# feldroop/genedex

Measured on AMD Instinct MI355X. Metric: queries/sec (count+locate), hg38-scale text, 100M len-50 reads, higher is better.
Workload: dtype u32

## Files before the change

### genedex_amd/csrc/search.hip

```cpp
#include <atomic>
#include <cstdlib>
#include <string>
#include <type_traits>

#include "common.hpp"
#include "kernels.hpp"

namespace gdx {

namespace {

constexpr int kBlock = 256;

struct QueryWindow {
    const uint64_t *words;
    uint64_t cur;
    uint64_t next;
    uint64_t cur_word;
    uint64_t first_word;

    __device__ __forceinline__ void init(const uint8_t *qbuf, uint64_t begin, uint64_t pos)
    {
        words = reinterpret_cast<const uint64_t *>(qbuf);
        first_word = begin >> 3;
// ... 1814 lines not shown
                    b[0] = a[0];
                    b[1] = a[1];
                }
                bool stepped = false;
                if (two) {
                    const uint32_t pair = (c2 - 1u) * 4u + (c1 - 1u);
                    const uint32_t bits_x = (c1 & 1u) | ((c1 & 2u) << 7) | ((c1 & 4u) << 14) | ((c2 & 1u) << 24);
                    const uint32_t bits_y = ((c2 >> 1) & 1u) | ((c2 & 4u) << 6);
                    const uint32_t nx = ~(bits_x * 0xffu);
                    const uint32_t ny = ~(bits_y * 0xffu) & 0xffffu;
                    uint32_t plo = 0, phi = 0;
#pragma unroll
                    for (int k = 0; k < 2; k++) {
                        plo += PairTable::pair_partial(a[k], sub + k * kGroup, pair, nx, ny, lo);
                        phi += PairTable::pair_partial(b[k], sub + k * kGroup, pair, nx, ny, hi);
                    }
                    const uint32_t nlo = quad_sum(plo), nhi = quad_sum(phi);
                    if (nlo != nhi) {
                        lo = nlo;
                        hi = nhi;
                        rem -= 2u;
                        part += 2u;
                        stepped = true;
                    }
                }
                if (!stepped) {
                    const uint32_t bits_x = (c1 & 1u) | ((c1 & 2u) << 7) | ((c1 & 4u) << 14);
                    const uint32_t nx = ~(bits_x * 0xffu) & 0xffffffu;
                    uint32_t plo = 0, phi = 0;
#pragma unroll
                    for (int k = 0; k < 2; k++) {
                        plo += PairTable::single_partial(a[k], sub + k * kGroup, c1, nx, lo);
                        phi += PairTable::single_partial(b[k], sub + k * kGroup, c1, nx, hi);
                    }
                    lo = quad_sum(plo);
                    hi = quad_sum(phi);
                    rem -= 1u;
                    part += 1u;
                }
                shift += part >> 3;
                part &= 7u;
            }
            if (writer) {
                if (bail) {
                    s_left[atomicAdd(&s_nleft, 1u)] = q;
                } else {
                    const bool unchanged = kCursor && len == 0u;
                    if (out_start && !unchanged) out_start[q] = lo;
                    if (out_end && !unchanged) out_end[q] = hi;
                    if (out_count) out_count[q] = hi - lo;
                    if (!kCursor && out_status) out_status[q] = 0;
                    if (kCursor && ca.active_out != nullptr && lo != hi && more_left) s_alive[slot] = q;
                }
            }
        }
        }
        __syncthreads();
        const uint32_t n_left = s_nleft;
        if (threadIdx.x == 0 && n_left != 0u) s_left_base = atomicAdd(n_leftover, n_left);
        __syncthreads();
        for (uint32_t i = threadIdx.x; i < n_left; i += kBlock) leftover[s_left_base + i] = s_left[i];
        __syncthreads();
        if (threadIdx.x == 0) s_nleft = 0;
        if (kCursor && ca.active_out != nullptr)
            flush_live_ordered(s_alive, cnt, s_alive_part, &s_alive_base, ca.active_out, ca.n_active_out);
    }
}

struct VerifyView {
    const uint2 *top;
    const u32x4 *text_units;
    const uint32_t *sa_full;
    const void *jump;
    const u32x4 *lines;
    const uint32_t *sb_offsets, *count, *sa_samples, *border_keys, *border_vals;
    const uint8_t *io_to_dense;
    uint32_t top_depth, n, n_texts, sa_inv, sa_rot, sa_limit, max_rows;
    uint32_t perm_code_lo, perm_code_hi, perm_exp_lo, perm_exp_hi, perm_mask;
    const u32x4 *seed;
    uint32_t seed_buckets, seed_k, seed_tag_bits;
    const u32x4 *seed_pairs, *seed_quads;
};

template <int kXlate, bool kSeed>
__global__ __launch_bounds__(kBlock) __attribute__((amdgpu_waves_per_eu(7, 7))) void search_verify_kernel4(
    VerifyView vv, const uint8_t *__restrict__ qbuf, const uint64_t *__restrict__ qbeg, const uint64_t *__restrict__ qend,
    uint64_t nq, uint32_t *__restrict__ out_count, uint8_t *__restrict__ out_status, uint4 *out_rec,
    uint32_t range, uint32_t *__restrict__ leftover, uint32_t *__restrict__ n_leftover,
    const uint32_t *__restrict__ list, const uint32_t *__restrict__ n_list,
    uint32_t ulen,
    const uint4 *state,
    uint32_t wide_to_list,
    uint32_t state_packed)
{
    constexpr int kGroup = 4;
    __shared__ uint8_t s_dense[256];
    __shared__ uint32_t s_count[8];
    __shared__ uint32_t s_left[kMaxRange];
    __shared__ uint32_t s_nleft, s_left_base;
    if (list != nullptr) nq = *n_list;
    if (static_cast<uint64_t>(blockIdx.x) * range >= nq) return;
    if (kXlate == 0)
        for (int i = threadIdx.x; i < 256; i += kBlock) s_dense[i] = vv.io_to_dense[i];
    if (threadIdx.x < 8) s_count[threadIdx.x] = threadIdx.x < 6 ? vv.count[threadIdx.x] : 0u;
    if (threadIdx.x == 0) s_nleft = 0;
    __syncthreads();
    IndexView ix{};
    ix.lines = vv.lines;
    ix.sb_offsets = vv.sb_offsets;
    ix.sa_inv = vv.sa_inv;
    ix.sa_rot = vv.sa_rot;
    ix.sa_limit = vv.sa_limit;
    const bool writer = (threadIdx.x % kGroup) == 0;
    const uint32_t sub = threadIdx.x & (kGroup - 1u);
    const uint32_t depth = vv.top_depth;
    const uint64_t n_ranges = (nq + range - 1) / range;
    for (uint64_t rg = blockIdx.x; rg < n_ranges; rg += gridDim.x) {
        const uint64_t base = rg * range;
        const uint32_t cnt = nq - base < range ? static_cast<uint32_t>(nq - base) : range;
        for (uint32_t slot = threadIdx.x / kGroup; slot < cnt; slot += kBlock / kGroup) {
            const uint32_t q = list != nullptr ? list[base + slot] : static_cast<uint32_t>(base + slot);
            uint4 st = make_uint4(0u, 0u, 0u, 0u);
            if (kSeed && state != nullptr) st = state[q];
            const bool from_state = kSeed && state != nullptr && state_packed != 0u && wide_to_list != 0u && (st.y & kStatePacked) != 0u &&
                                    (st.y & kStateSymbolsMask) <= 32u;
            const uint64_t begin = from_state ? 0ull : query_begin(qbeg, ulen, q);
            const uint64_t len = from_state ? 0ull : query_end(qend, ulen, q) - begin;
            bool bail = from_state ? false
                                   : (kSeed ? !(len >= vv.seed_k && len < (1ull << 21)) : !(len >= 16u && len >= depth && len < (1ull << 21)));
            uint32_t lo = 0, hi = 0, rem = 0;
            const uint64_t *wbase = query_words<kXlate>(qbuf, begin);
            const uint32_t off0 = static_cast<uint32_t>(begin & 7u);
            FastWindow w = {0u, 0u, 0u, 0u, 0u, 8u};
            uint32_t shift = 0, part = 0;
            bool single = false;
            bool single_ok = false;
            uint32_t pos = 0;
            bool resumed = false;
            const uint64_t state_codes = (static_cast<uint64_t>(st.z) << 32) | st.w;
            if (from_state && (st.y & kStatePair) != 0u && (st.y >> kStateRowsShift) > 2u) {
                const u32x4 *qr = vv.seed_quads + 4ull * st.x;
                const u32x4 q0 = qr[0], q1 = qr[1], q2 = qr[2], q3 = qr[3];
                const uint32_t n_v = st.y & kStateSymbolsMask, rows_q = st.y >> kStateRowsShift;
                const uint64_t vm64 = n_v == 32u ? ~0ull : ~0ull << (2u * (32u - n_v));
                const uint32_t p_me = sel4(sub, q0.x, q0.y, q0.z, q0.w);
                const uint64_t t_me = (static_cast<uint64_t>(sel4(sub, q1.y, q1.w, q2.y, q2.w)) << 32) | sel4(sub, q1.x, q1.z, q2.x, q2.z);
                uint32_t alive_q = (sub < rows_q && ((state_codes ^ t_me) & vm64) == 0ull && p_me >= n_v) ? 1u << sub : 0u;
                alive_q |= static_cast<uint32_t>(__builtin_amdgcn_mov_dpp(static_cast<int>(alive_q), 0xB1, 0xF, 0xF, true));
                alive_q |= static_cast<uint32_t>(__builtin_amdgcn_mov_dpp(static_cast<int>(alive_q), 0x4E, 0xF, 0xF, true));
                if (writer) {
                    const uint32_t n_alive = static_cast<uint32_t>(__popc(alive_q));
                    uint4 rec;
                    if (n_alive == 0u) {
                        rec = make_uint4(0u, 0u, 0xffffffffu, 0u);
                    } else if (n_alive <= 2u) {
                        const uint32_t f = static_cast<uint32_t>(__builtin_ctz(alive_q));
                        const uint32_t h1 = sel4(f, q0.x, q0.y, q0.z, q0.w) - n_v;
                        if (n_alive == 1u) {
                            rec = make_uint4(0u, 1u, h1, kRecResolved);
                        } else {
                            const uint32_t g = static_cast<uint32_t>(__builtin_ctz(alive_q & (alive_q - 1u)));
                            const uint32_t h2 = sel4(g, q0.x, q0.y, q0.z, q0.w) - n_v;
                            rec = make_uint4(h2, h2 + 2u, h1, kRecResolved);
                        }
                    } else {
                        rec = make_uint4(q3.x, q3.x + n_alive, alive_q, (n_v & 0x1fffffu) | kRecMasked);
                    }
                    if (out_rec) out_rec[q] = rec;
                    if (out_count) out_count[q] = rec.y - rec.x;
                    if (out_status) out_status[q] = 0;
                }
                continue;
            }
            if (from_state && (st.y & kStatePair) != 0u) {
                const u32x4 *pr = vv.seed_pairs + 2ull * st.x;
                const u32x4 r0 = pr[0], r1 = pr[1];
                const uint32_t n_v = st.y & kStateSymbolsMask;
                const uint64_t vm64 = n_v == 32u ? ~0ull : ~0ull << (2u * (32u - n_v));
                const uint64_t t1 = (static_cast<uint64_t>(r0.w) << 32) | r0.z, t2 = (static_cast<uint64_t>(r1.y) << 32) | r1.x;
                const bool ok1 = ((state_codes ^ t1) & vm64) == 0ull && r0.x >= n_v, ok2 = ((state_codes ^ t2) & vm64) == 0ull && r0.y >= n_v;
                if (writer) {
                    const uint32_t h1 = r0.x - n_v, h2 = r0.y - n_v;
                    uint4 rec;
                    if (ok1 && ok2) rec = make_uint4(h2, h2 + 2u, h1, kRecResolved);
                    else if (ok1 || ok2) rec = make_uint4(0u, 1u, ok1 ? h1 : h2, kRecResolved);
                    else rec = make_uint4(0u, 0u, 0xffffffffu, 0u);
                    if (out_rec) out_rec[q] = rec;
                    if (out_count) out_count[q] = rec.y - rec.x;
                    if (out_status) out_status[q] = 0;
                }
                continue;
            }
            if (from_state) {
                resumed = true;
                lo = st.x;
                hi = lo + (st.y >> kStateRowsShift);
                rem = st.y & kStateSymbolsMask;
            } else if (kSeed && !bail && state != nullptr) {
                const bool plain = state_packed == 0u && st.w == 1u;
                const bool p_rows = state_packed != 0u && (st.y & kStatePacked) != 0u, p_wide = state_packed != 0u && (st.y & kStatePlain) != 0u;
                if (plain || p_rows || p_wide) {
                    resumed = true;
                    rem = static_cast<uint32_t>(len);
                    w = fast_window<kXlate>(vv, s_dense, wbase, off0, rem, sub);
                    lo = st.x;
                    hi = plain ? st.y : (p_rows ? lo + (st.y >> kStateRowsShift) : st.z);
                    rem = plain ? st.z : st.y & kStateSymbolsMask;
                    shift = vv.seed_k >> 3;
                    part = vv.seed_k & 7u;
                }
            }
            if (kSeed && !bail && !resumed) {
                rem = static_cast<uint32_t>(len);
                w = fast_window<kXlate>(vv, s_dense, wbase, off0, rem, sub);
                const uint32_t k = vv.seed_k;
                const uint32_t n_look = rem < k + 32u ? rem : k + 32u;
                const uint32_t n_words = n_look <= w.s0 ? 1u : 1u + ((n_look - w.s0 + 7u) >> 3);
                if ((w.valid8 & ((1u << n_words) - 1u)) != (1u << n_words) - 1u) {
                    bail = true;
                } else {
                    const uint32_t w0 = __builtin_amdgcn_alignbit(w.l0, w.l0, 16), w1 = __builtin_amdgcn_alignbit(w.l1, w.l1, 16);
                    const uint32_t w2 = __builtin_amdgcn_alignbit(w.l2, w.l2, 16), w3 = __builtin_amdgcn_alignbit(w.l3, w.l3, 16);
                    const uint64_t key = ((static_cast<uint64_t>(w0) << 32) | w1) >> (64u - 2u * k);
                    uint32_t tag;
                    uint32_t b = seed_home(key, vv.seed_tag_bits, vv.seed_buckets, tag);
                    uint32_t ex, ey, ez, ew;
                    for (uint32_t d = 0;; d++) {
                        const u32x4 *bp = vv.seed + (static_cast<uint64_t>(b) << 3) + 2u * sub;
                        const u32x4 e0 = bp[0], e1 = bp[1];
                        const uint32_t want = tag | (d << kSeedDispShift);
                        const bool m0 = (e0.x & kSeedMatchMask) == want, m1 = (e1.x & kSeedMatchMask) == want;
                        const u32x4 es = m0 ? e0 : e1;
                        const bool m = m0 || m1;
                        ex = m ? (es.x | kSeedFound) : (e0.x & kSeedOverflow);
                        ey = m ? es.y : 0u;
                        ez = m ? es.z : 0u;
                        ew = m ? es.w : 0u;
                        ex |= static_cast<uint32_t>(__builtin_amdgcn_mov_dpp(static_cast<int>(ex), 0xB1, 0xF, 0xF, true));
                        ey |= static_cast<uint32_t>(__builtin_amdgcn_mov_dpp(static_cast<int>(ey), 0xB1, 0xF, 0xF, true));
                        ez |= static_cast<uint32_t>(__builtin_amdgcn_mov_dpp(static_cast<int>(ez), 0xB1, 0xF, 0xF, true));
                        ew |= static_cast<uint32_t>(__builtin_amdgcn_mov_dpp(static_cast<int>(ew), 0xB1, 0xF, 0xF, true));
                        ex |= static_cast<uint32_t>(__builtin_amdgcn_mov_dpp(static_cast<int>(ex), 0x4E, 0xF, 0xF, true));
                        ey |= static_cast<uint32_t>(__builtin_amdgcn_mov_dpp(static_cast<int>(ey), 0x4E, 0xF, 0xF, true));
                        ez |= static_cast<uint32_t>(__builtin_amdgcn_mov_dpp(static_cast<int>(ez), 0x4E, 0xF, 0xF, true));
                        ew |= static_cast<uint32_t>(__builtin_amdgcn_mov_dpp(static_cast<int>(ew), 0x4E, 0xF, 0xF, true));
                        if ((ex & kSeedFound) != 0u || (ex & kSeedOverflow) == 0u || d >= kSeedMaxDisp) break;
                        b = b + 1u == vv.seed_buckets ? 0u : b + 1u;
                    }
                    rem -= k;
                    shift = k >> 3;
                    part = k & 7u;
                    if ((ex & kSeedFound) == 0u) {
                        lo = hi = 0u;
                    } else if ((ex & kSeedKind) != 0u) {
                        lo = ey;
                        hi = ez;
                    } else {
                        single = true;
                        lo = 0u;
                        hi = 1u;
                        pos = ey;
                        uint32_t qh, ql;
                        const uint32_t sh = 32u - 2u * (k & 15u);
                        if (k == 16u) {
                            qh = w1;
                            ql = w2;
                        } else if (k < 16u) {
                            qh = __builtin_amdgcn_alignbit(w0, w1, sh);
                            ql = __builtin_amdgcn_alignbit(w1, w2, sh);
                        } else {
                            qh = __builtin_amdgcn_alignbit(w1, w2, sh);
                            ql = __builtin_amdgcn_alignbit(w2, w3, sh);
                        }
// ... 820 lines not shown
                    const uint32_t n_need = (static_cast<uint32_t>(at & 7u) + n_c + 7u) >> 3;
                    uint64_t lo64 = up[0];
                    uint32_t hi16 = 0;
                    if (n_need > 1u) lo64 |= static_cast<uint64_t>(up[1]) << 16;
                    if (n_need > 2u) lo64 |= static_cast<uint64_t>(up[2]) << 32;
                    if (n_need > 3u) lo64 |= static_cast<uint64_t>(up[3]) << 48;
                    if (n_need > 4u) hi16 = up[4];
                    u0 = tu[0];
                    u1 = tb != 0u ? tu[1] : u32x4{0u, 0u, 0u, 0u};
                    qc = sh != 0u ? (lo64 >> sh) | (static_cast<uint64_t>(hi16) << (64u - sh)) : lo64;
                } else {
                const uint64_t *wp = reinterpret_cast<const uint64_t *>(qbuf) + (at >> 3);
                const uint32_t sh = static_cast<uint32_t>(at & 7u) * 8u;
                const uint32_t n_need = (static_cast<uint32_t>(at & 7u) + n_c + 7u) >> 3;
                uint64_t w0 = wp[0], w1 = 0, w2 = 0, w3 = 0, w4 = 0;
                if (n_need > 1u) w1 = wp[1];
                if (n_need > 2u) w2 = wp[2];
                if (n_need > 3u) w3 = wp[3];
                if (n_need > 4u) w4 = wp[4];
                u0 = tu[0];
                u1 = tb != 0u ? tu[1] : u32x4{0u, 0u, 0u, 0u};
                if (sh != 0u) {
                    w0 = (w0 >> sh) | (w1 << (64u - sh));
                    w1 = (w1 >> sh) | (w2 << (64u - sh));
                    w2 = (w2 >> sh) | (w3 << (64u - sh));
                    w3 = (w3 >> sh) | (w4 << (64u - sh));
                }
                uint32_t b[8] = {0u, 0u, 0u, 0u, 0u, 0u, 0u, 0u};
                const uint32_t wd[8] = {static_cast<uint32_t>(w0), static_cast<uint32_t>(w0 >> 32), static_cast<uint32_t>(w1),
                                        static_cast<uint32_t>(w1 >> 32), static_cast<uint32_t>(w2), static_cast<uint32_t>(w2 >> 32),
                                        static_cast<uint32_t>(w3), static_cast<uint32_t>(w3 >> 32)};
#pragma unroll
                for (uint32_t g = 0; g < 8; g++) {
                    const uint32_t code = kXlate == 1 ? fast_pack4(sv, wd[g], b[g]) : fast_pack4_lds(s_dense, wd[g], b[g]);
                    qc |= static_cast<uint64_t>(code) << (8u * g);
                }
                const uint32_t full = n_c >> 2, part = n_c & 3u;
#pragma unroll
                for (uint32_t g = 0; g < 8; g++) {
                    const uint32_t bg = kXlate == 1 ? b[g] : (b[g] != 0u ? 0xffffffffu : 0u);
                    if (g < full) inv |= bg;
                    else if (g == full && part != 0u) inv |= bg & ((1u << (8u * part)) - 1u);
                }
                }
                const uint64_t c0 = static_cast<uint64_t>(u0.x) | (static_cast<uint64_t>(u0.y) << 32);
                const uint64_t c1 = static_cast<uint64_t>(u1.x) | (static_cast<uint64_t>(u1.y) << 32);
                const uint64_t tc = tb ? (c0 >> (2u * tb)) | (c1 << (64u - 2u * tb)) : c0;
                const uint32_t tm = tb ? (u0.z >> tb) | (u1.z << (32u - tb)) : u0.z;
                const uint64_t m64 = n_c == 32u ? ~0ull : (1ull << (2u * n_c)) - 1ull;
                const uint32_t m32 = n_c == 32u ? ~0u : (1u << n_c) - 1u;
                if (inv != 0u) bad_q = 1u;
                if (((qc ^ tc) & m64) != 0ull || (tm & m32) != 0u) bad_t = 1u;
            }
        }
        const bool left = group_max<kGroup>(bad_q) != 0u;
        const bool hit = group_max<kGroup>(bad_t) == 0u;
        if (kExact) {
            if (left || !hit) {
                if (writer) leftover[atomicAdd(n_leftover, 1u)] = q;
            } else {
                const uint32_t row = sv.isa[pos - rem];
                if (writer) {
                    out_start[q] = row;
                    out_end[q] = row + 1u;
                    if (out_count) out_count[q] = 1u;
                    if (out_status) out_status[q] = 0;
                }
            }
        } else if (writer) {
            if (left) {
                leftover[atomicAdd(n_leftover, 1u)] = q;
                if (state) state[q] = make_uint4(0u, 0u, 0u, 0u);
                if (out_compact) out_compact[q] = kCompactSee;
            } else {
                if (out_compact) out_compact[q] = hit ? pos - rem : kCompactNone;
                else if (out_rec) out_rec[q] = hit ? make_uint4(0u, 1u, pos - rem, kRecResolved) : make_uint4(0u, 0u, 0xffffffffu, 0u);
                if (out_count) out_count[q] = hit ? 1u : 0u;
                if (out_status) out_status[q] = 0;
            }
        }
    }
}

template <int kJump, int kMode>
__global__ __launch_bounds__(kBlock) __attribute__((amdgpu_waves_per_eu(7, 7))) void search_pair_packed_kernel4(GDX_SEARCH_ARGS)
{
    search_pair_body<0, 4, false, kJump, kMode, true>(GDX_SEARCH_FWD);
}
template <int kPolicy, int kJump, int kMode>
__global__ __launch_bounds__(kBlock) void search_pair_stats_kernel8(GDX_SEARCH_ARGS)
{
    search_pair_body<kPolicy, 8, true, kJump, kMode>(GDX_SEARCH_FWD);
}
template <int kPolicy, int kJump, int kMode>
__global__ __launch_bounds__(kBlock) void search_pair_stats_kernel4(GDX_SEARCH_ARGS)
{
    search_pair_body<kPolicy, 4, true, kJump, kMode>(GDX_SEARCH_FWD);
}

template <class Table, int kGroup, bool kPair>
__global__ __launch_bounds__(kBlock) void extend_front_kernel(IndexView ix, uint32_t *__restrict__ start,
                                                              uint32_t *__restrict__ end,
                                                              const uint8_t *__restrict__ io_symbols, uint64_t m,
                                                              uint8_t *__restrict__ out_status)
{
    const uint64_t stride = static_cast<uint64_t>(gridDim.x) * (kBlock / kGroup);
    const bool writer = (threadIdx.x % kGroup) == 0;
    for (uint64_t i = static_cast<uint64_t>(blockIdx.x) * (kBlock / kGroup) + threadIdx.x / kGroup; i < m; i += stride) {
        uint32_t lo = start[i], hi = end[i];
        const uint32_t c = ix.io_to_dense[io_symbols[i]];
        uint32_t status = GDX_Q_OK;
        if (c == 0) {
            status = GDX_Q_INVALID_SYMBOL;
        } else if (lo != hi) {
            if (kPair && c <= 4u) {
                PairTable::lf1<1, 8>(ix, c, lo, hi, lo, hi);
            } else {
                uint32_t rlo, rhi;
                Table::rank2(ix, c, lo, hi, rlo, rhi);
                const uint32_t cc = ix.count[c];
                lo = cc + rlo;
                hi = cc + rhi;
            }
            if (writer) {
                start[i] = lo;
                end[i] = hi;
            }
        }
        if (out_status && writer) out_status[i] = static_cast<uint8_t>(status);
    }
}

struct SegmentsOut {
    uint32_t *n_segments, *remaining, *length, *start, *end;
    uint8_t *status;
};

template <class Table, int kGroup, bool kPair, bool kText>
__global__ __launch_bounds__(kBlock) __attribute__((amdgpu_waves_per_eu((kText && kPair) ? 5 : ((kText || kGroup == 1) ? 6 : 7)))) void suffix_segments_kernel(
    IndexView ix, const uint8_t *__restrict__ qbuf, const uint64_t *__restrict__ qoff, uint64_t nq, uint32_t max_segments,
    SegmentsOut out)
{
    __shared__ uint8_t s_dense[256];
    __shared__ uint32_t s_count[257];
    for (int i = threadIdx.x; i < 256; i += kBlock) s_dense[i] = ix.io_to_dense[i];
    for (int i = threadIdx.x; i <= ix.sigma; i += kBlock) s_count[i] = ix.count[i];
    __syncthreads();

    const uint64_t stride = static_cast<uint64_t>(gridDim.x) * (kBlock / kGroup);
    const bool writer = (threadIdx.x % kGroup) == 0;
    const uint32_t sub = threadIdx.x % kGroup;
    const uint32_t depth = (ix.top != nullptr && ix.layout == 0) ? ix.top_depth : 0u;
    for (uint64_t q = static_cast<uint64_t>(blockIdx.x) * (kBlock / kGroup) + threadIdx.x / kGroup; q < nq; q += stride) {
        const uint64_t begin = qoff[q];
        const uint32_t m = static_cast<uint32_t>(qoff[q + 1] - begin);
        const uint64_t slot0 = q * max_segments;
        uint32_t e = m, n_seg = 0, status = GDX_Q_OK;
        while (e > 0u && n_seg < max_segments) {
            uint32_t lo = 0, hi = ix.n, len = 0;
            if (depth != 0u && e >= depth) {
                uint32_t a = 0, b = 0;
                for (uint32_t s = 0; s < depth; s++) {
                    const uint32_t c = s_dense[qbuf[begin + e - 1u - s]];
                    if (s < 8u) a |= c << (4u * (7u - s));
                    else b |= c << (4u * (15u - s));
                }
// ... 575 lines not shown
    const uint64_t ranges = (nq + range - 1) / range;
    return static_cast<unsigned>(ranges < cap ? ranges : cap);
}
static ListGrid range_grid(uint64_t nq, uint32_t range_cap, long grid_override)
{
    uint64_t per_block = (nq + 1791) / 1792;
    per_block = (per_block + 63) / 64 * 64;
    const uint32_t range = static_cast<uint32_t>(per_block > range_cap ? range_cap : per_block);
    return {grid_override > 0 ? static_cast<unsigned>(grid_override) : range_blocks(nq, range, 1u << 20), range};
}
static ListGrid short_list_grid(uint64_t nq, unsigned cap = 8192) { return {range_blocks(nq, 256, cap), 256}; }
static unsigned group_grid(uint64_t nq, uint64_t groups_per_block, long grid_override)
{
    const uint64_t needed = (nq + groups_per_block - 1) / groups_per_block;
    uint64_t blocks = (nq + groups_per_block * 48 - 1) / (groups_per_block * 48);
    if (blocks < 1792) blocks = 1792;
    if (blocks > 65536) blocks = 65536;
    if (blocks > needed) blocks = needed;
    if (grid_override > 0) blocks = static_cast<uint64_t>(grid_override);
    return static_cast<unsigned>(blocks);
}

static SeedView seed_view(const IndexView &ix, const uint32_t *isa)
{
    return SeedView{ix.seed, ix.text_units, isa, ix.io_to_dense, ix.seed_buckets, ix.seed_k, ix.seed_tag_bits,
                    ix.perm_code_lo, ix.perm_code_hi, ix.perm_exp_lo, ix.perm_exp_hi, ix.perm_mask};
}
static VerifyView verify_view(const IndexView &ix)
{
    const bool entry_sa = ix.jump != nullptr && ix.jump_bytes == 32;
    const uint32_t max_rows = (ix.sa_full != nullptr || entry_sa) ? 4u : 1u;
    return VerifyView{ix.top, ix.text_units, ix.sa_full, entry_sa ? ix.jump : nullptr, ix.lines, ix.sb_offsets, ix.count,
                      ix.sa_samples, ix.border_keys, ix.border_vals, ix.io_to_dense, ix.top_depth, ix.n, ix.n_texts,
                      ix.sa_inv, ix.sa_rot, ix.sa_limit, max_rows, ix.perm_code_lo, ix.perm_code_hi, ix.perm_exp_lo,
                      ix.perm_exp_hi, ix.perm_mask, ix.seed, ix.seed_buckets, ix.seed_k, ix.seed_tag_bits, ix.seed_pairs, ix.seed_quads};
}
static ExactView exact_view(const IndexView &ix, bool with_seed)
{
    return ExactView{ix.top, ix.jump, ix.pair_lines, ix.io_to_dense, ix.top_depth, ix.n, static_cast<uint32_t>(ix.depth),
                     ix.perm_code_lo, ix.perm_code_hi, ix.perm_exp_lo, ix.perm_exp_hi, ix.perm_mask, ix.sa_full, ix.isa,
                     ix.text_units, with_seed ? ix.seed : nullptr, ix.seed_buckets, ix.seed_k, ix.seed_tag_bits};
}
static FastView fast_view(const IndexView &ix)
{
    return FastView{ix.top, ix.jump, ix.io_to_dense, ix.top_depth, ix.sa_inv, ix.sa_rot, ix.sa_limit,
                    ix.perm_code_lo, ix.perm_code_hi, ix.perm_exp_lo, ix.perm_exp_hi, ix.perm_mask};
}

struct SeedLaunch {
    SeedView sv;
    ListGrid grid;
    unsigned lds = 0;
    uint4 *rec = nullptr;
    uint32_t *start = nullptr, *end = nullptr;
    uint32_t *first = nullptr, *lng = nullptr;
    uint4 *state = nullptr;
    uint32_t *compact = nullptr;
    uint2 *long_state = nullptr;
    uint32_t long_stride = 0, state_packed = 0;
};

struct SearchChain {
    ZeroSet zs;
    CursorArgs ca;
    bool leftover_list = false;
    uint32_t *seed_list = nullptr;
    uint32_t seed_state_packed = 0;
    bool compact_by_seed = false;
    uint32_t *fold_left = nullptr, *fold_long = nullptr;
    uint64_t *d_uniform_off = nullptr;
    bool sparse_offsets = false;
    ListGrid all{}, exact{}, general{};
    CursorArgs ca_exact, ca_general;
};

struct SearchLauncher {
    const IndexView &ix;
    SearchCall c;
    hipStream_t stream;
    const SearchKnobs &k;
    const SearchSettings s;
    const uint64_t nq;
    const bool seed_pairs;
    const long lane_blocks_cap;
    uint32_t ulen = 0;
    SearchChain st;

    uint32_t *counted_list(int slot, ZeroSet *zs)
    {
        uint32_t *list = static_cast<uint32_t *>(stream_scratch(stream, slot, (nq + 4) * sizeof(uint32_t)));
        if (zs != nullptr) zs->add(list, sizeof(uint32_t));
        else GDX_HIP(hipMemsetAsync(list, 0, sizeof(uint32_t), stream));
        return list;
    }
    void print_left(const char *path, const uint32_t *n_list, const char *next)
    {
        uint32_t n_left = 0;
        GDX_HIP(hipMemcpyAsync(&n_left, n_list, sizeof(uint32_t), hipMemcpyDeviceToHost, stream));
        GDX_HIP(hipStreamSynchronize(stream));
        fprintf(stderr, "gdx: %s path left %u of %llu queries to the %s kernel\n", path, n_left, static_cast<unsigned long long>(nq), next);
    }
    template <int kXlate, bool kExact>
    void launch_seed_text(const SeedLaunch &a)
    {
        hipLaunchKernelGGL((seed_text_kernel4<kXlate, kExact>), dim3(range_blocks(nq, kBlock / 4, 8192)), dim3(kBlock), 0, stream, a.sv,
                           c.d_qbuf, c.d_qbeg, a.lng + 4, a.lng, a.long_state, a.long_stride, c.d_count, c.d_status, a.rec, a.start,
                           a.end, a.compact, a.state, a.first + 4, a.first, ulen);
    }
    template <int kXlate, bool kExact>
    void launch_seed_and_text(const SeedLaunch &a)
    {
        hipLaunchKernelGGL((search_seed_kernel4<kXlate, kExact>), dim3(a.grid.blocks), dim3(kBlock), a.lds, stream, a.sv, c.d_qbuf,
                           c.d_qbeg, c.d_qend, nq, c.d_count, c.d_status, a.rec, a.start, a.end, a.grid.range, a.first + 4, a.first,
                           a.state, a.compact, a.lng + 4, a.lng, a.long_state, a.long_stride, a.state_packed, ulen, CursorArgs());
        launch_seed_text<kXlate, kExact>(a);
    }
    template <bool kSeed>
    void launch_verify(ListGrid grid, uint32_t *left, uint32_t *list, const uint4 *state, uint32_t wide)
    {
        const VerifyView vv = verify_view(ix);
        with_xlate(s.xlate, [&](auto X) {
            hipLaunchKernelGGL((search_verify_kernel4<decltype(X)::value, kSeed>), dim3(grid.blocks), dim3(kBlock), 0, stream, vv,
                               c.d_qbuf, c.d_qbeg, c.d_qend, nq, c.d_count, c.d_status, c.d_rec, grid.range, left + 4, left,
                               list ? list + 4 : nullptr, list, ulen, state, wide, state != nullptr ? st.seed_state_packed : 0u);
        });
    }

    void seed_front(ListGrid v_grid, uint32_t *d_left)
    {
        const bool pair_general = s.variant == 2 && ix.pair_lines != nullptr;
        const bool to_fast = k.seed_lean != 0 && k.seed_chain != 0 && pair_general && ix.top != nullptr && ix.top_depth >= 1u &&
                             ix.jump != nullptr && ix.top_depth >= static_cast<uint32_t>(ix.depth) && s.lanes == 4 && s.policy == 0 &&
                             s.fast != 0;
        const bool to_verify_packed = !to_fast && pair_general && k.seed_lean != 0;
        st.seed_state_packed = (to_fast || to_verify_packed) && c.d_rec != nullptr && k.seed_packed != 0 ? 1u : 0u;
        if (st.seed_state_packed != 0u && !to_fast && (ix.seed_pairs != nullptr || ix.seed_quads != nullptr) && seed_pairs)
            st.seed_state_packed = 2u;
        if (k.seed_lean == 0) {
            st.zs.flush(stream);
            return launch_verify<true>(v_grid, d_left, nullptr, nullptr, 0u);
        }
        SeedLaunch a{seed_view(ix, nullptr), v_grid, k.seed_pad, c.d_rec};
        a.first = counted_list(12, &st.zs);
        const bool to_verify_with_state = !to_fast && pair_general && c.d_rec != nullptr;
        a.state = (to_fast || to_verify_with_state) ? c.d_rec : nullptr;
        a.compact = c.d_compact;
        a.lng = counted_list(13, &st.zs);
        a.long_state = c.d_rec != nullptr ? reinterpret_cast<uint2 *>(c.d_rec) : static_cast<uint2 *>(stream_scratch(stream, 14, nq * sizeof(uint2)));
        a.long_stride = c.d_rec != nullptr ? 2u : 1u;
        a.state_packed = st.seed_state_packed;
        const bool lane_kernel = k.seed_lane != 0 && s.xlate != 0 && ix.seed_k <= 24u && ix.seed_k >= 8u &&
                                 (reinterpret_cast<uintptr_t>(c.d_qbuf) & 3u) == 0;
        unsigned long long *fold = nullptr;
        if (lane_kernel && c.d_tile_sums != nullptr && c.d_tile_rest != nullptr && c.d_compact != nullptr) {
            fold = c.d_tile_sums;
            st.zs.add(fold, ((nq + kSumTile - 1) / kSumTile) * sizeof(unsigned long long));
            st.fold_left = a.first;
            st.fold_long = a.lng;
        }
        const uint32_t lane_range = k.seed_lane_range >= 64u && k.seed_lane_range <= kLaneRange ? k.seed_lane_range / 64u * 64u
                                    : (v_grid.range < kLaneRange ? v_grid.range : kLaneRange);
        if (lane_range % 64u != 0u) fail(GDX_ERR_INVALID_ARGUMENT, "internal: the lane kernel's ranges are multiples of 64");
        unsigned lane_blocks = range_blocks(nq, lane_range, 1u << 20);
        if (lane_blocks_cap > 0 && static_cast<unsigned long>(lane_blocks_cap) < lane_blocks) lane_blocks = static_cast<unsigned>(lane_blocks_cap);
        st.zs.flush(stream);
        if (lane_kernel) {
            with_int<2, 1>(s.xlate, [&](auto X) {
                constexpr int kX = decltype(X)::value;
                with_bool(ulen != 0u, [&](auto U) {
                    hipLaunchKernelGGL((search_seed_lane_kernel<kX, decltype(U)::value>), dim3(lane_blocks), dim3(kBlock), a.lds, stream,
                                       a.sv, c.d_qbuf, c.d_qbeg, c.d_qend, nq, c.d_count, c.d_status, c.d_rec, lane_range, a.first + 4,
                                       a.first, a.state, a.compact, a.lng + 4, a.lng, a.long_state, a.long_stride, a.state_packed, ulen, fold);
                });
                launch_seed_text<kX, false>(a);
            });
        } else {
            with_xlate(s.xlate, [&](auto X) { launch_seed_and_text<decltype(X)::value, false>(a); });
        }
        st.compact_by_seed = true;
        if (to_fast) {
            st.seed_list = a.first;
            return;
        }
        if (to_verify_with_state) st.ca.resume_state = a.state;
        launch_verify<true>(short_list_grid(nq, k.seed_list_blocks), d_left, a.first, to_verify_with_state ? a.state : nullptr,
                            to_verify_with_state ? 1u : 0u);
    }

    void front()
    {
        const bool clean_call = c.mode == 1 && ix.layout == 0 && ix.text_units != nullptr && ix.n_searchable >= 4 &&
                                c.d_step_stats == nullptr && c.d_hint == nullptr && c.d_start == nullptr &&
                                c.d_end == nullptr && st.ca.active_in == nullptr && nq < 0xffffffffull;
        const bool seed = clean_call && ix.seed != nullptr && ix.seed_k >= static_cast<uint32_t>(ix.depth) && s.seed;
        const bool verify = !seed && clean_call && ix.top != nullptr && ix.top_depth >= 1u && ix.jump == nullptr &&
                            ix.top_depth >= static_cast<uint32_t>(ix.depth) && s.fast != 0;
        if (!seed && !verify) return;
        const ListGrid v_grid = range_grid(nq, kMaxRange, 0);
        uint32_t *d_left = counted_list(11, &st.zs);
        if (seed) {
            seed_front(v_grid, d_left);
        } else {
            st.zs.flush(stream);
            launch_verify<false>(v_grid, d_left, nullptr, nullptr, 0u);
        }
        uint32_t *next = st.seed_list ? st.seed_list : d_left;
        if (k.fast_stats) print_left(seed ? "seed" : "verify", next, "next");
        st.ca.active_in = next + 4;
        st.ca.n_active_in = next;
        st.leftover_list = true;
    }

    void uniform_offsets(bool sparse)
    {
        st.d_uniform_off = static_cast<uint64_t *>(stream_scratch(stream, 15, (nq + 1) * sizeof(uint64_t)));
        if (!sparse)
            hipLaunchKernelGGL(fill_uniform_offsets_kernel, dim3(grid_for_items(nq + 1)), dim3(kBlock), 0, stream, st.d_uniform_off,
                               nq + 1, c.uniform_len);
        c.d_qbeg = st.d_uniform_off;
        c.d_qend = st.d_uniform_off + 1;
        c.uniform_len = 0;
        st.sparse_offsets = sparse;
    }
    void offsets_for_list(const uint32_t *list, const uint32_t *n_list)
    {
        if (st.sparse_offsets && list != nullptr)
            hipLaunchKernelGGL(fill_uniform_offsets_list_kernel, dim3(1024), dim3(kBlock), 0, stream, st.d_uniform_off, list, n_list, ulen);
    }

    void pair_seed_exact()
    {
        SeedLaunch a{seed_view(ix, ix.isa), st.all};
        a.first = counted_list(12, nullptr);
        a.start = c.d_start;
        a.end = c.d_end;
        a.lng = counted_list(13, nullptr);
        with_xlate(s.xlate, [&](auto X) { launch_seed_and_text<decltype(X)::value, true>(a); });
        st.ca_exact.active_in = a.first + 4;
        st.ca_exact.n_active_in = a.first;
        st.exact = short_list_grid(nq);
    }
    void pair_seed_cursor()
    {
        uint32_t *d_first = counted_list(12, nullptr);
        SeedView sv = seed_view(ix, ix.isa);
        sv.n = ix.n;
        with_int<1, 0>(s.perm ? 1 : 0, [&](auto X) {
            hipLaunchKernelGGL((search_seed_kernel4<decltype(X)::value, true, true>), dim3(st.all.blocks), dim3(kBlock), 0, stream, sv,
                               c.d_qbuf, c.d_qbeg, c.d_qend, nq, c.d_count, c.d_status, nullptr, c.d_start, c.d_end, st.all.range,
                               d_first + 4, d_first, nullptr, nullptr, nullptr, nullptr, nullptr, 0u, 0u, 0u, st.ca);
        });
        st.ca_exact.active_in = d_first + 4;
        st.ca_exact.n_active_in = d_first;
        st.exact = short_list_grid(nq);
    }
    void pair_exact(bool seed_in_kernel)
    {
        uint32_t *d_left = counted_list(11, nullptr);
        const ExactView ev = exact_view(ix, seed_in_kernel);
        auto launch = [&](auto kernel) {
            hipLaunchKernelGGL(kernel, dim3(st.exact.blocks), dim3(kBlock), 0, stream, ev, c.d_qbuf, c.d_qbeg, c.d_qend, nq, c.d_start,
                               c.d_end, c.d_count, c.d_status, st.exact.range, s.schedule, d_left + 4, d_left, st.ca_exact);
        };
        if (s.text_route && c.packed) launch(search_exact_kernel4<0, 2, false, true>);
        else
            with_bool(c.mode == 2, [&](auto C) {
                constexpr bool kCursor = decltype(C)::value;
                with_int<1, 0>(s.perm ? 1 : 0, [&](auto X) {
// ... 44 lines not shown
        with_jump_bytes(ix.jump_bytes, [&](auto J) {
            constexpr int kJ = decltype(J)::value;
            if (c.packed) {
                with_int<0, 1>(c.mode, [&](auto M) { launch(search_pair_packed_kernel4<kJ, decltype(M)::value>); });
            } else if (c.d_step_stats != nullptr) {
                launch(lanes8 ? search_pair_stats_kernel8<0, kJ, 0> : search_pair_stats_kernel4<0, kJ, 0>);
            } else if (s.defer_after != 0u && c.mode != 2) {
                with_int<0, 1>(c.mode, [&](auto M) {
                    constexpr int kM = decltype(M)::value;
                    launch(lanes8 ? search_pair_defer_kernel8<0, kJ, kM> : search_pair_defer_kernel4<0, kJ, kM>);
                });
            } else {
                with_int<0, 1>(s.policy, [&](auto P) {
                    constexpr int kP = decltype(P)::value;
                    with_int<0, 1, 2>(c.mode, [&](auto M) {
                        constexpr int kM = decltype(M)::value;
                        launch(lanes8 ? search_pair_kernel8<kP, kJ, kM> : search_pair_kernel4<kP, kJ, kM>);
                    });
                });
            }
        });
    }
    void pair_lines()
    {
        const CursorArgs &ca = st.ca;
        const bool lanes4_plain = s.lanes == 4 && s.policy == 0;
        st.all = range_grid(nq, c.mode == 2 ? kCursorRange : kMaxRange, k.grid);
        const bool fast = c.mode == 1 && c.d_step_stats == nullptr && lanes4_plain &&
                          ix.top != nullptr && ix.top_depth >= 1u && ix.jump != nullptr &&
                          ix.n_searchable >= 4 && ix.top_depth >= static_cast<uint32_t>(ix.depth) &&
                          (ca.active_in == nullptr || st.seed_list != nullptr) && c.d_hint == nullptr && c.d_start == nullptr &&
                          c.d_end == nullptr && s.fast != 0 && nq < 0xffffffffull;
        if (st.seed_list != nullptr && !fast) fail(GDX_ERR_INVALID_ARGUMENT, "internal: the seed kernel's list without the fast kernel");
        st.ca_general = ca;
        st.general = st.leftover_list ? short_list_grid(nq) : st.all;
        const bool exact = (c.mode == 0 || c.mode == 2) && c.d_step_stats == nullptr && lanes4_plain &&
                           (!c.packed || (c.mode == 0 && s.text_route)) &&
                           c.d_hint == nullptr && c.d_rec == nullptr && c.d_start != nullptr && c.d_end != nullptr &&
                           ix.n_searchable >= 4 && ix.sigma >= 5 && ca.resume_state == nullptr &&
                           (ix.top == nullptr || ix.top_depth >= static_cast<uint32_t>(ix.depth)) &&
                           s.exact && (s.defer_after == 0u || c.mode == 2) && nq < 0xffffffffull;
        st.ca_exact = ca;
        st.exact = st.all;
        const bool seed_exact = exact && c.mode == 0 && ix.seed != nullptr && ix.isa != nullptr && ix.text_units != nullptr &&
                                ix.seed_k >= static_cast<uint32_t>(ix.depth) && ca.active_in == nullptr && s.seed;
        if (seed_exact) pair_seed_exact();
        const bool seed_usable = ix.seed != nullptr && ix.seed_k >= static_cast<uint32_t>(ix.depth) && ix.seed_k <= 24u;
        const bool seed_cursor = exact && c.mode == 2 && s.text_route && seed_usable && k.seed_cursor != 0 && s.seed &&
                                 (ca.chunk_symbols != 0u ? (ca.chunk_index == 0u && ca.chunk_symbols >= ix.seed_k && ca.chunk_symbols <= ix.seed_k + 32u)
                                                         : ca.active_in == nullptr);
        if (seed_cursor) pair_seed_cursor();
        if (exact) pair_exact(seed_usable && !seed_cursor);
        if (fast) pair_fast();
        offsets_for_list(st.ca_general.active_in, st.ca_general.n_active_in);
        pair_general();
    }

    template <class Table, int kGroup>
    void launch_plain(unsigned grid)
    {
        auto launch = [&](auto kernel) {
            hipLaunchKernelGGL(kernel, dim3(grid), dim3(kBlock), k.pad, stream, ix, c.d_qbuf, c.d_qbeg, c.d_qend, nq, c.d_start, c.d_end,
                               c.d_count, c.d_status, c.d_step_stats, c.d_rec, st.ca, ulen);
        };
        if (c.mode == 2) launch(search_kernel<Table, kGroup, true>);
        else if (c.packed) launch(search_kernel<Table, kGroup, false, true>);
        else launch(search_kernel<Table, kGroup, false>);
    }
    void finish_fold()
    {
        if (st.fold_left == nullptr) return;
        hipLaunchKernelGGL(tile_sums_lists_kernel, dim3(4096), dim3(kBlock), 0, stream, c.d_rec, c.d_compact, c.tile_max_hits,
                           st.fold_left + 4, st.fold_left, st.fold_long + 4, st.fold_long, c.d_tile_sums, c.d_tile_rest);
        if (c.tile_sums_done != nullptr) *c.tile_sums_done = true;
    }
};

void launch_search_call(const IndexView &ix, const SearchCall &call, hipStream_t stream, const QueryOptions &qo)
{
    if (call.nq == 0) return;
    if (call.mode < 0 || call.mode > 2) fail(GDX_ERR_INVALID_ARGUMENT, "internal: search mode %d", call.mode);
    const SearchKnobs &knobs = search_knobs();
    const char *env_pairs = getenv("GDX_SEARCH_SEED_PAIRS");
    const char *env_lane_blocks = getenv("GDX_SEED_LANE_BLOCKS");
    SearchLauncher l{ix, call, stream, knobs, SearchSettings(ix, qo, knobs, call), call.nq,
                     !(env_pairs != nullptr && atoi(env_pairs) == 0), env_lane_blocks != nullptr ? atol(env_lane_blocks) : 0L};
    SearchCall &c = l.c;
    if (c.packed) check_packed_supported(ix);
    if (c.packed && (c.mode == 2 || c.d_step_stats != nullptr)) fail(GDX_ERR_UNSUPPORTED, "packed queries: search and count / locate only");
    const bool pair_lines = ix.layout == 0 && l.s.variant == 2 && ix.pair_lines != nullptr;
    const bool pair_offsets = c.uniform_len != 0u && pair_lines;
    if (pair_offsets && c.mode != 1) l.uniform_offsets(false);
    l.ulen = c.uniform_len;
    if (c.also_zero != nullptr) l.st.zs = *c.also_zero;
    l.st.ca = c.cursors;
    if (c.tile_sums_done != nullptr) *c.tile_sums_done = false;
    if (c.d_compact != nullptr && (c.mode != 1 || c.d_rec == nullptr))
        fail(GDX_ERR_INVALID_ARGUMENT, "internal: compact results go with the records of a count / locate search");
    l.front();
    l.st.zs.flush(stream);
    if (pair_offsets && c.mode == 1) l.uniform_offsets(l.st.leftover_list);
    if (c.d_compact != nullptr && !l.st.compact_by_seed)
        GDX_HIP(hipMemsetD32Async(reinterpret_cast<hipDeviceptr_t>(c.d_compact), static_cast<int>(kCompactSee), l.nq, stream));
    if (pair_lines) {
        l.pair_lines();
    } else {
        if (c.d_hint) GDX_HIP(hipMemsetAsync(c.d_hint, 0xff, l.nq * sizeof(uint2), stream));
        if (ix.layout == 0 && l.s.variant != 1) l.launch_plain<QuadLineTable, 4>(group_grid(l.nq, kBlock / 4, knobs.grid));
        else if (ix.layout == 0) l.launch_plain<LineTable, 1>(grid_for_items(l.nq));
        else l.launch_plain<GenericTable, 1>(grid_for_items(l.nq));
    }
    l.finish_fold();
}

__global__ __launch_bounds__(kBlock) void pack_queries_kernel(const uint8_t *__restrict__ io_to_dense,
                                                              const uint8_t *__restrict__ qbuf, uint64_t n_symbols,
                                                              uint8_t *__restrict__ packed, uint8_t *__restrict__ bad_flags,
                                                              unsigned long long *__restrict__ bad_symbols)
{
    __shared__ uint8_t s_dense[256];
    for (int i = threadIdx.x; i < 256; i += kBlock) s_dense[i] = io_to_dense[i];
    __syncthreads();
    const uint64_t n_bytes = (n_symbols + 3) / 4;
    const uint64_t stride = static_cast<uint64_t>(gridDim.x) * kBlock;
    uint32_t bad = 0;
    for (uint64_t b = static_cast<uint64_t>(blockIdx.x) * kBlock + threadIdx.x; b < n_bytes; b += stride) {
        uint32_t out = 0;
#pragma unroll
        for (uint32_t k = 0; k < 4; k++) {
            const uint64_t j = 4 * b + k;
            if (j < n_symbols) {
                const uint32_t d = s_dense[qbuf[j]];
                if (d - 1u < 4u) {
                    out |= (d - 1u) << (2u * k);
                } else {
                    bad++;
                    if (bad_flags) bad_flags[j >> 6] = 1;
                }
            }
        }
        packed[b] = static_cast<uint8_t>(out);
    }
    if (bad && bad_symbols) atomicAdd(bad_symbols, static_cast<unsigned long long>(bad));
}

void launch_pack_queries(const IndexView &ix, const uint8_t *d_qbuf, uint64_t n_symbols, uint8_t *d_packed,
                         uint8_t *d_bad_flags, unsigned long long *d_bad_symbols, hipStream_t stream)
{
    if (n_symbols == 0) return;
    hipLaunchKernelGGL(pack_queries_kernel, dim3(grid_for_items((n_symbols + 3) / 4)), dim3(kBlock), 0, stream,
                       ix.io_to_dense, d_qbuf, n_symbols, d_packed, d_bad_flags, d_bad_symbols);
}

void launch_extend_front(const IndexView &ix, uint32_t *d_start, uint32_t *d_end, const uint8_t *d_io_symbols,
                         uint64_t m, uint8_t *d_out_status, hipStream_t stream)
{
    if (m == 0) return;
    if (ix.layout == 0 && ix.pair_lines != nullptr) {
        hipLaunchKernelGGL((extend_front_kernel<QuadLineTable, 8, true>), dim3(grid_for_items(m * 8)), dim3(kBlock), 0,
                           stream, ix, d_start, d_end, d_io_symbols, m, d_out_status);
    } else if (ix.layout == 0) {
        hipLaunchKernelGGL((extend_front_kernel<QuadLineTable, 4, false>), dim3(grid_for_items(m * 4)), dim3(kBlock), 0,
                           stream, ix, d_start, d_end, d_io_symbols, m, d_out_status);
    } else {
        hipLaunchKernelGGL((extend_front_kernel<GenericTable, 1, false>), dim3(grid_for_items(m)), dim3(kBlock), 0,
                           stream, ix, d_start, d_end, d_io_symbols, m, d_out_status);
    }
}

// ... 100 lines not shown
```

Before: 26.63 billion.

## Resolve seed pair/quad records in a dedicated light kernel before verify

Adds a seed_records_kernel that walks the seed list and resolves queries whose packed state already points at a pair or quad record, writing their results directly. The remaining queries are compacted into a new leftover list, which is then passed to the heavy verify kernel. The aim is to stop decided queries from occupying the register-heavy verify kernel's slots and diverging within its groups. The cost is an extra kernel launch, one more list round trip through memory and an atomic per block. Shared record-decoding helpers are factored out for both paths, and an environment variable allows disabling the new kernel.

```diff
diff --git a/genedex_amd/csrc/search.hip b/genedex_amd/csrc/search.hip
--- a/genedex_amd/csrc/search.hip
+++ b/genedex_amd/csrc/search.hip
@@ -1920,6 +1920,53 @@
     const u32x4 *seed_pairs, *seed_quads;
 };
 
+__device__ __forceinline__ uint64_t record_front_mask(uint32_t n_v) { return n_v == 32u ? ~0ull : ~0ull << (2u * (32u - n_v)); }
+__device__ __forceinline__ bool record_row_survives(uint64_t codes, uint64_t context, uint64_t vm64, uint32_t p, uint32_t n_v)
+{
+    return ((codes ^ context) & vm64) == 0ull && p >= n_v;
+}
+__device__ __forceinline__ uint32_t quad_row_position(u32x4 q0, uint32_t r) { return sel4(r, q0.x, q0.y, q0.z, q0.w); }
+__device__ __forceinline__ uint64_t quad_row_context(u32x4 q1, u32x4 q2, uint32_t r)
+{
+    return (static_cast<uint64_t>(sel4(r, q1.y, q1.w, q2.y, q2.w)) << 32) | sel4(r, q1.x, q1.z, q2.x, q2.z);
+}
+__device__ __forceinline__ uint4 pair_rows_record(bool ok1, bool ok2, uint32_t p1, uint32_t p2, uint32_t n_v)
+{
+    const uint32_t h1 = p1 - n_v, h2 = p2 - n_v;
+    uint4 rec;
+    if (ok1 && ok2) rec = make_uint4(h2, h2 + 2u, h1, kRecResolved);
+    else if (ok1 || ok2) rec = make_uint4(0u, 1u, ok1 ? h1 : h2, kRecResolved);
+    else rec = make_uint4(0u, 0u, 0xffffffffu, 0u);
+    return rec;
+}
+__device__ __forceinline__ uint4 quad_rows_record(uint32_t alive_q, u32x4 q0, uint32_t lo, uint32_t n_v)
+{
+    const uint32_t n_alive = static_cast<uint32_t>(__popc(alive_q));
+    uint4 rec;
+    if (n_alive == 0u) {
+        rec = make_uint4(0u, 0u, 0xffffffffu, 0u);
+    } else if (n_alive <= 2u) {
+        const uint32_t f = static_cast<uint32_t>(__builtin_ctz(alive_q));
+        const uint32_t h1 = quad_row_position(q0, f) - n_v;
+        if (n_alive == 1u) {
+            rec = make_uint4(0u, 1u, h1, kRecResolved);
+        } else {
+            const uint32_t g = static_cast<uint32_t>(__builtin_ctz(alive_q & (alive_q - 1u)));
+            const uint32_t h2 = quad_row_position(q0, g) - n_v;
+            rec = make_uint4(h2, h2 + 2u, h1, kRecResolved);
+        }
+    } else {
+        rec = make_uint4(lo, lo + n_alive, alive_q, (n_v & 0x1fffffu) | kRecMasked);
+    }
+    return rec;
+}
+__device__ __forceinline__ void store_decided(uint32_t q, uint4 rec, uint32_t *out_count, uint8_t *out_status, uint4 *out_rec)
+{
+    if (out_rec) out_rec[q] = rec;
+    if (out_count) out_count[q] = rec.y - rec.x;
+    if (out_status) out_status[q] = 0;
+}
+
 template <int kXlate, bool kSeed>
 __global__ __launch_bounds__(kBlock) __attribute__((amdgpu_waves_per_eu(7, 7))) void search_verify_kernel4(
     VerifyView vv, const uint8_t *__restrict__ qbuf, const uint64_t *__restrict__ qbeg, const uint64_t *__restrict__ qend,
@@ -1980,53 +2027,22 @@
                 const u32x4 *qr = vv.seed_quads + 4ull * st.x;
                 const u32x4 q0 = qr[0], q1 = qr[1], q2 = qr[2], q3 = qr[3];
                 const uint32_t n_v = st.y & kStateSymbolsMask, rows_q = st.y >> kStateRowsShift;
-                const uint64_t vm64 = n_v == 32u ? ~0ull : ~0ull << (2u * (32u - n_v));
-                const uint32_t p_me = sel4(sub, q0.x, q0.y, q0.z, q0.w);
-                const uint64_t t_me = (static_cast<uint64_t>(sel4(sub, q1.y, q1.w, q2.y, q2.w)) << 32) | sel4(sub, q1.x, q1.z, q2.x, q2.z);
-                uint32_t alive_q = (sub < rows_q && ((state_codes ^ t_me) & vm64) == 0ull && p_me >= n_v) ? 1u << sub : 0u;
+                const uint64_t vm64 = record_front_mask(n_v);
+                uint32_t alive_q = (sub < rows_q && record_row_survives(state_codes, quad_row_context(q1, q2, sub), vm64,
+                                                                        quad_row_position(q0, sub), n_v)) ? 1u << sub : 0u;
                 alive_q |= static_cast<uint32_t>(__builtin_amdgcn_mov_dpp(static_cast<int>(alive_q), 0xB1, 0xF, 0xF, true));
                 alive_q |= static_cast<uint32_t>(__builtin_amdgcn_mov_dpp(static_cast<int>(alive_q), 0x4E, 0xF, 0xF, true));
-                if (writer) {
-                    const uint32_t n_alive = static_cast<uint32_t>(__popc(alive_q));
-                    uint4 rec;
-                    if (n_alive == 0u) {
-                        rec = make_uint4(0u, 0u, 0xffffffffu, 0u);
-                    } else if (n_alive <= 2u) {
-                        const uint32_t f = static_cast<uint32_t>(__builtin_ctz(alive_q));
-                        const uint32_t h1 = sel4(f, q0.x, q0.y, q0.z, q0.w) - n_v;
-                        if (n_alive == 1u) {
-                            rec = make_uint4(0u, 1u, h1, kRecResolved);
-                        } else {
-                            const uint32_t g = static_cast<uint32_t>(__builtin_ctz(alive_q & (alive_q - 1u)));
-                            const uint32_t h2 = sel4(g, q0.x, q0.y, q0.z, q0.w) - n_v;
-                            rec = make_uint4(h2, h2 + 2u, h1, kRecResolved);
-                        }
-                    } else {
-                        rec = make_uint4(q3.x, q3.x + n_alive, alive_q, (n_v & 0x1fffffu) | kRecMasked);
-                    }
-                    if (out_rec) out_rec[q] = rec;
-                    if (out_count) out_count[q] = rec.y - rec.x;
-                    if (out_status) out_status[q] = 0;
-                }
+                if (writer) store_decided(q, quad_rows_record(alive_q, q0, q3.x, n_v), out_count, out_status, out_rec);
                 continue;
             }
             if (from_state && (st.y & kStatePair) != 0u) {
                 const u32x4 *pr = vv.seed_pairs + 2ull * st.x;
                 const u32x4 r0 = pr[0], r1 = pr[1];
                 const uint32_t n_v = st.y & kStateSymbolsMask;
-                const uint64_t vm64 = n_v == 32u ? ~0ull : ~0ull << (2u * (32u - n_v));
+                const uint64_t vm64 = record_front_mask(n_v);
                 const uint64_t t1 = (static_cast<uint64_t>(r0.w) << 32) | r0.z, t2 = (static_cast<uint64_t>(r1.y) << 32) | r1.x;
-                const bool ok1 = ((state_codes ^ t1) & vm64) == 0ull && r0.x >= n_v, ok2 = ((state_codes ^ t2) & vm64) == 0ull && r0.y >= n_v;
-                if (writer) {
-                    const uint32_t h1 = r0.x - n_v, h2 = r0.y - n_v;
-                    uint4 rec;
-                    if (ok1 && ok2) rec = make_uint4(h2, h2 + 2u, h1, kRecResolved);
-                    else if (ok1 || ok2) rec = make_uint4(0u, 1u, ok1 ? h1 : h2, kRecResolved);
-                    else rec = make_uint4(0u, 0u, 0xffffffffu, 0u);
-                    if (out_rec) out_rec[q] = rec;
-                    if (out_count) out_count[q] = rec.y - rec.x;
-                    if (out_status) out_status[q] = 0;
-                }
+                const bool ok1 = record_row_survives(state_codes, t1, vm64, r0.x, n_v), ok2 = record_row_survives(state_codes, t2, vm64, r0.y, n_v);
+                if (writer) store_decided(q, pair_rows_record(ok1, ok2, r0.x, r0.y, n_v), out_count, out_status, out_rec);
                 continue;
             }
             if (from_state) {
@@ -3013,6 +3029,77 @@
     }
 }
 
+constexpr uint32_t kRecordsRange = 2048;
+__global__ __launch_bounds__(kBlock) __attribute__((amdgpu_waves_per_eu(8, 8))) void seed_records_kernel(
+    const u32x4 *__restrict__ seed_pairs, const u32x4 *__restrict__ seed_quads, const uint32_t *__restrict__ list,
+    const uint32_t *__restrict__ n_list, const uint4 *state,
+    uint32_t *__restrict__ out_count, uint8_t *__restrict__ out_status, uint4 *out_rec, uint32_t *__restrict__ rest,
+    uint32_t *__restrict__ n_rest)
+{
+    constexpr uint32_t kWaves = kBlock / 64, kPerWave = kRecordsRange / kWaves;
+    static_assert(kPerWave % 64 == 0, "a wavefront takes whole chunks of 64 entries");
+    __shared__ uint32_t s_rest[kWaves][kPerWave];
+    __shared__ uint32_t s_n[kWaves], s_base;
+    const uint64_t n = *n_list;
+    if (static_cast<uint64_t>(blockIdx.x) * kRecordsRange >= n) return;
+    const uint32_t lane = threadIdx.x & 63u, wave = threadIdx.x >> 6;
+    const uint64_t n_ranges = (n + kRecordsRange - 1) / kRecordsRange;
+    for (uint64_t rg = blockIdx.x; rg < n_ranges; rg += gridDim.x) {
+        const uint64_t base = rg * kRecordsRange + wave * kPerWave;
+        uint32_t n_mine = 0;
+        for (uint32_t it = 0; it < kPerWave && base + it < n; it += 64u) {
+            const uint64_t i = base + it + lane;
+            const bool live = i < n;
+            const uint32_t q = live ? list[i] : 0u;
+            uint4 st = make_uint4(0u, 0u, 0u, 0u);
+            if (live) st = state[q];
+            const bool decided = live && (st.y & (kStatePacked | kStatePair)) == (kStatePacked | kStatePair) && (st.y & kStateSymbolsMask) <= 32u;
+            if (decided) {
+                const uint32_t rows = st.y >> kStateRowsShift, n_v = st.y & kStateSymbolsMask;
+                const bool quad = rows > 2u;
+                const u32x4 *rp = quad ? seed_quads + 4ull * st.x : seed_pairs + 2ull * st.x;
+                const u32x4 a0 = rp[0], a1 = rp[1];
+                u32x4 a2 = {0u, 0u, 0u, 0u};
+                uint32_t lo = 0;
+                if (quad) {
+                    a2 = rp[2];
+                    lo = reinterpret_cast<const uint32_t *>(rp + 3)[0];
+                }
+                const uint64_t codes = (static_cast<uint64_t>(st.z) << 32) | st.w, vm64 = record_front_mask(n_v);
+                uint4 rec;
+                if (quad) {
+                    uint32_t alive_q = 0;
+#pragma unroll
+                    for (uint32_t r = 0; r < 4; r++)
+                        if (r < rows && record_row_survives(codes, quad_row_context(a1, a2, r), vm64, quad_row_position(a0, r), n_v)) alive_q |= 1u << r;
+                    rec = quad_rows_record(alive_q, a0, lo, n_v);
+                } else {
+                    const uint64_t t1 = (static_cast<uint64_t>(a0.w) << 32) | a0.z, t2 = (static_cast<uint64_t>(a1.y) << 32) | a1.x;
+                    rec = pair_rows_record(record_row_survives(codes, t1, vm64, a0.x, n_v), record_row_survives(codes, t2, vm64, a0.y, n_v),
+                                           a0.x, a0.y, n_v);
+                }
+                store_decided(q, rec, out_count, out_status, out_rec);
+            }
+            const bool hand_on = live && !decided;
+            const unsigned long long mask = __ballot(hand_on);
+            if (hand_on) s_rest[wave][n_mine + static_cast<uint32_t>(__popcll(mask & ((1ull << lane) - 1ull)))] = q;
+            n_mine += static_cast<uint32_t>(__popcll(mask));
+        }
+        if (lane == 0u) s_n[wave] = n_mine;
+        __syncthreads();
+        if (threadIdx.x == 0) {
+            uint32_t total = 0;
+            for (uint32_t w = 0; w < kWaves; w++) total += s_n[w];
+            s_base = total != 0u ? atomicAdd(n_rest, total) : 0u;
+        }
+        __syncthreads();
+        uint32_t at = s_base;
+        for (uint32_t w = 0; w < wave; w++) at += s_n[w];
+        for (uint32_t j = lane; j < n_mine; j += 64u) rest[at + j] = s_rest[wave][j];
+        __syncthreads();
+    }
+}
+
 template <int kJump, int kMode>
 __global__ __launch_bounds__(kBlock) __attribute__((amdgpu_waves_per_eu(7, 7))) void search_pair_packed_kernel4(GDX_SEARCH_ARGS)
 {
@@ -3754,6 +3841,7 @@
     const SearchSettings s;
     const uint64_t nq;
     const bool seed_pairs;
+    const bool records_kernel;
     const long lane_blocks_cap;
     uint32_t ulen = 0;
     SearchChain st;
@@ -3834,6 +3922,7 @@
                                     : (v_grid.range < kLaneRange ? v_grid.range : kLaneRange);
         if (lane_range % 64u != 0u) fail(GDX_ERR_INVALID_ARGUMENT, "internal: the lane kernel's ranges are multiples of 64");
         unsigned lane_blocks = range_blocks(nq, lane_range, 1u << 20);
+        uint32_t *rest = st.seed_state_packed == 2u && records_kernel ? counted_list(16, &st.zs) : nullptr;
         if (lane_blocks_cap > 0 && static_cast<unsigned long>(lane_blocks_cap) < lane_blocks) lane_blocks = static_cast<unsigned>(lane_blocks_cap);
         st.zs.flush(stream);
         if (lane_kernel) {
@@ -3855,7 +3944,10 @@
             return;
         }
         if (to_verify_with_state) st.ca.resume_state = a.state;
-        launch_verify<true>(short_list_grid(nq, k.seed_list_blocks), d_left, a.first, to_verify_with_state ? a.state : nullptr,
+        if (rest != nullptr)
+            hipLaunchKernelGGL(seed_records_kernel, dim3(range_blocks(nq, kRecordsRange, 2048)), dim3(kBlock), 0, stream, ix.seed_pairs,
+                               ix.seed_quads, a.first + 4, a.first, a.state, c.d_count, c.d_status, c.d_rec, rest + 4, rest);
+        launch_verify<true>(short_list_grid(nq, k.seed_list_blocks), d_left, rest != nullptr ? rest : a.first, to_verify_with_state ? a.state : nullptr,
                             to_verify_with_state ? 1u : 0u);
     }
 
@@ -4066,9 +4158,11 @@
     if (call.mode < 0 || call.mode > 2) fail(GDX_ERR_INVALID_ARGUMENT, "internal: search mode %d", call.mode);
     const SearchKnobs &knobs = search_knobs();
     const char *env_pairs = getenv("GDX_SEARCH_SEED_PAIRS");
+    const char *env_records_kernel = getenv("GDX_SEARCH_SEED_RECORDS_KERNEL");
     const char *env_lane_blocks = getenv("GDX_SEED_LANE_BLOCKS");
     SearchLauncher l{ix, call, stream, knobs, SearchSettings(ix, qo, knobs, call), call.nq,
-                     !(env_pairs != nullptr && atoi(env_pairs) == 0), env_lane_blocks != nullptr ? atol(env_lane_blocks) : 0L};
+                     !(env_pairs != nullptr && atoi(env_pairs) == 0), !(env_records_kernel != nullptr && atoi(env_records_kernel) == 0),
+                     env_lane_blocks != nullptr ? atol(env_lane_blocks) : 0L};
     SearchCall &c = l.c;
     if (c.packed) check_packed_supported(ix);
     if (c.packed && (c.mode == 2 || c.d_step_stats != nullptr)) fail(GDX_ERR_UNSUPPORTED, "packed queries: search and count / locate only");
```

Result: slower. 26.08 billion (-2.1%).
